# fegemo/palette-and-histo-gan

Measured on AMD Instinct MI355X. Metric: train images/sec (64x64x4 sprites), higher is better.
Workload: dtype bf16

## Files before the change

palette_and_histo_gan_amd/csrc/norm_act.hip:

```cpp
#include "p2p_common.hpp"
#include <stdlib.h>

#include <type_traits>

typedef __attribute__((__vector_size__(2 * sizeof(float)))) float f32x2;

__device__ __forceinline__ float act_apply(float y, int act, float alpha) {
    if (act == P2P_ACT_LEAKY) return y > 0.f ? y : alpha * y;
    if (act == P2P_ACT_RELU) return y > 0.f ? y : 0.f;
    return y;
}
__device__ __forceinline__ float act_slope(float a, int act, float alpha) {
    if (act == P2P_ACT_LEAKY) return a > 0.f ? 1.f : alpha;
    if (act == P2P_ACT_RELU) return a > 0.f ? 1.f : 0.f;
    return 1.f;
}

template <int VN> using mask_word = typename std::conditional<VN == 8, unsigned long long, unsigned>::type;
template <int VN>
__device__ __forceinline__ mask_word<VN> mask_vload(const unsigned char* m) { return *(const mask_word<VN>*)m; }
template <typename M>
__device__ __forceinline__ float mask_keep(M mk, int k) { return ((mk >> (8 * k)) & 0xff) ? 2.f : 0.f; }
template <int VN>
__device__ __forceinline__ void mask_vkeep(const unsigned char* m, float* keep) {
    const mask_word<VN> mk = mask_vload<VN>(m);
#pragma unroll
    for (int k = 0; k < VN; ++k) keep[k] = mask_keep(mk, k);
}

__device__ __forceinline__ float norm_xhat(float x, float mu, float rs) { return (x - mu) * rs; }

__device__ __forceinline__ float norm_affine(float x, float mu, float rs, float ga, float be) { return norm_xhat(x, mu, rs) * ga + be; }
__device__ __forceinline__ float drop_act(float y, bool drop, float keep, int act, float alpha) {
    if (drop) y *= keep;
    return act_apply(y, act, alpha);
}
__device__ __forceinline__ float fwd_elem(float x, float mu, float rs, float ga, float be, bool drop, float keep, int act, float alpha) {
    return drop_act(norm_affine(x, mu, rs, ga, be), drop, keep, act, alpha);
}

__device__ __forceinline__ float bwd_elem(bool norm, float xh, float ga, float be, float keep, float da, int act, float alpha) {
    float a = norm ? xh * ga + be : xh;
    a *= keep;
    return da * act_slope(a, act, alpha) * keep;
}
__device__ __forceinline__ float bwd_dx(float ga, float rs, float d, float m1, float xh, float m2) { return ga * rs * (d - m1 - xh * m2); }

template <typename T>
__device__ __forceinline__ float raw_load(const void* raw, int raw_kind, int nslabs, long long slab, long long e) {
    if (raw_kind == 1) return to_f32(((const T*)raw)[e]);
    float s = 0.f;
    const float* p = (const float*)raw + e;
    for (int k = 0; k < nslabs; ++k) s += p[(long long)k * slab];
    return to_f32(from_f32<T>(s));
}

template <typename T>
__global__ void norm_act_fwd_kernel(int H, int W, int C, int CB, const void* __restrict__ raw, int raw_kind,
// ... 151 lines not shown
#pragma unroll
        for (int u = 0; u < 4; ++u)
#pragma unroll
            for (int k = 0; k < VN; k += 4) r[u][k / 4] = *(const f32x4*)(p + (long long)(sIdx + u) * slab + k);
#pragma unroll
        for (int u = 0; u < 4; ++u)
#pragma unroll
            for (int k = 0; k < VN; k += 4) {
                v[k] += r[u][k / 4][0]; v[k + 1] += r[u][k / 4][1]; v[k + 2] += r[u][k / 4][2]; v[k + 3] += r[u][k / 4][3];
            }
    }
    return sIdx;
}

template <typename T, int SLABS = 1>
__device__ __forceinline__ void raw_vload(const void* raw, int raw_kind, int nslabs, long long slab, long long e, float* v) {
    constexpr int VN = VecOf<T>::N;
    if (SLABS == 0 || raw_kind == 1) { vload<T>((const T*)raw + e, v); return; }
#pragma unroll
    for (int k = 0; k < VN; ++k) v[k] = 0.f;
    const float* p = (const float*)raw + e;
    int sIdx = SLABS == 4 ? slabs4_add<VN>(p, slab, nslabs, v) : 0;
    for (; sIdx < nslabs; ++sIdx) {
#pragma unroll
        for (int k = 0; k < VN; k += 4) {
            f32x4 r = *(const f32x4*)(p + (long long)sIdx * slab + k);
            v[k] += r[0]; v[k + 1] += r[1]; v[k + 2] += r[2]; v[k + 3] += r[3];
        }
    }
#pragma unroll
    for (int k = 0; k < VN; ++k) v[k] = to_f32(from_f32<T>(v[k]));
}

template <typename T, int SLABS = 1>
__device__ __forceinline__ void gsrc_vload(const GSrc& g, long long pix, int c, float* v) {
    constexpr int VN = VecOf<T>::N;
    if (g.kind == 0) {
#pragma unroll
        for (int k = 0; k < VN; ++k) v[k] = 0.f;
        return;
    }
    long long e = pix * g.ld + g.coff + c;
    if (SLABS == 0 || g.kind == 1) { vload<T>((const T*)g.ptr + e, v); return; }
#pragma unroll
    for (int k = 0; k < VN; ++k) v[k] = 0.f;
    const float* p = (const float*)g.ptr + e;
    int sIdx = 0;
    if (SLABS == 4 && (g.slab & 3) == 0 && (e & 3) == 0 && ((uintptr_t)g.ptr & 15) == 0) sIdx = slabs4_add<VN>(p, g.slab, g.nslabs, v);
    for (; sIdx < g.nslabs; ++sIdx)
#pragma unroll
        for (int k = 0; k < VN; ++k) v[k] += p[(long long)sIdx * g.slab + k];
}

template <int VN> struct Coef { float mu[VN], rs[VN], ga[VN], be[VN]; };

template <int VN>
__device__ __forceinline__ void coef_load(const float* stats, const float* gamma, const float* beta, int n, int C, int c, Coef<VN>& co) {
#pragma unroll
    for (int k = 0; k < VN; ++k) {
        co.mu[k] = stats[((long long)n * C + c + k) * 2 + 0];
        co.rs[k] = stats[((long long)n * C + c + k) * 2 + 1];
        co.ga[k] = gamma[c + k];
        co.be[k] = beta[c + k];
    }
}

template <int VN>
__device__ __forceinline__ void coef_from_sums(const float* t1, const float* t2, const float* sh, int HW, float eps, const float* gamma,
                                               const float* beta, float* stats, bool write, int n, int C, int c, Coef<VN>& co) {
#pragma unroll
    for (int k = 0; k < VN; ++k) {
        const float m = t1[k] / (float)HW;
        const float var = fmaxf(t2[k] / (float)HW - m * m, 0.f);
        co.mu[k] = sh[k] + m;
        co.rs[k] = rsqrtf(var + eps);
        co.ga[k] = gamma[c + k];
        co.be[k] = beta[c + k];
        if (write) {
            stats[((long long)n * C + c + k) * 2 + 0] = co.mu[k];
            stats[((long long)n * C + c + k) * 2 + 1] = co.rs[k];
        }
    }
}

template <int VN> struct WgGeom {
    int VPP, PR, vid, pr, c;
    __device__ __forceinline__ WgGeom(int CG, int cg0)
        : VPP(CG / VN), PR(256 / VPP), vid(threadIdx.x % VPP), pr(threadIdx.x / VPP), c(cg0 + vid * VN) {}
};

template <int VN, bool TREE = false>
__device__ __forceinline__ void col_reduce2(float (*red)[2048], int CG, int PR, int vid, int pr, const float* s1,
                                            const float* s2, float* t1, float* t2) {
#pragma unroll
    for (int k = 0; k < VN; k += 4) {
        *(f32x4*)&red[0][pr * CG + vid * VN + k] = f32x4{s1[k], s1[k + 1], s1[k + 2], s1[k + 3]};
        *(f32x4*)&red[1][pr * CG + vid * VN + k] = f32x4{s2[k], s2[k + 1], s2[k + 2], s2[k + 3]};
    }
    __syncthreads();
    const int Q = 256 / CG;
    const int ch = threadIdx.x % CG, q = threadIdx.x / CG;
    float a = 0.f, b = 0.f;
    if (TREE) {
        float ra[VN], rb[VN];
#pragma unroll
        for (int j = 0; j < VN; ++j) { ra[j] = red[0][(q + j * Q) * CG + ch]; rb[j] = red[1][(q + j * Q) * CG + ch]; }
#pragma unroll
        for (int w = 1; w < VN; w *= 2)
#pragma unroll
            for (int j = 0; j < VN; j += 2 * w) { ra[j] += ra[j + w]; rb[j] += rb[j + w]; }
        a = ra[0]; b = rb[0];
    } else {
        for (int i = q; i < PR; i += Q) { a += red[0][i * CG + ch]; b += red[1][i * CG + ch]; }
    }
    __syncthreads();
    red[0][q * CG + ch] = a;
    red[1][q * CG + ch] = b;
    __syncthreads();
    if (threadIdx.x < CG) {
        float ta = 0.f, tb = 0.f;
        if (TREE) {
            float fa[8], fb[8];
#pragma unroll
            for (int g = 0; g < 8; ++g) {
                fa[g] = 0.f; fb[g] = 0.f;
                if (8 * g < Q) {
                    const float* pa = &red[0][8 * g * CG + threadIdx.x];
                    const float* pb = &red[1][8 * g * CG + threadIdx.x];
                    fa[g] = (pa[0] + pa[CG]) + (pa[2 * CG] + pa[3 * CG]);
                    fb[g] = (pb[0] + pb[CG]) + (pb[2 * CG] + pb[3 * CG]);
// ... 28 lines not shown
    }
}
template <int VN>
__device__ __forceinline__ void split_sum(const float* ws, float (*red)[2048], int n, int SP, int C, int cg0, int CG, int vid,
                                          float* t1, float* t2) {
    if (threadIdx.x < CG) {
        const int cc = cg0 + threadIdx.x;
        float a1 = 0.f, a2 = 0.f;
        for (int i = 0; i < SP; ++i) {
            const f32x2 v = *(const f32x2*)(ws + (((long long)n * SP + i) * C + cc) * 2);
            a1 += v[0]; a2 += v[1];
        }
        red[0][threadIdx.x] = a1;
        red[1][threadIdx.x] = a2;
    }
    __syncthreads();
#pragma unroll
    for (int k = 0; k < VN; ++k) { t1[k] = red[0][vid * VN + k]; t2[k] = red[1][vid * VN + k]; }
}

template <typename T>
__device__ __forceinline__ void tail_copy(T* dst, const T* src, int t0, int tail_vecs) {
    typedef typename VecOf<T>::type vec_t;
    for (int t = t0; t < tail_vecs; ++t) *(vec_t*)(dst + t * VecOf<T>::N) = *(const vec_t*)(src + t * VecOf<T>::N);
}

template <typename T, int MODE>
__global__ __launch_bounds__(256) void norm_act_fwd_vec(int H, int W, int C, int CG, const void* __restrict__ raw,
                                                        int raw_kind, int nslabs, long long slab,
                                                        const float* __restrict__ gamma, const float* __restrict__ beta,
                                                        float eps, int act, float alpha,
                                                        const unsigned char* __restrict__ mask, TView out,
                                                        T* __restrict__ raw_out, float* __restrict__ stats,
                                                        float* __restrict__ ws, int nslots, TView tail, int tail_vecs) {
    constexpr int VN = VecOf<T>::N;
    __shared__ __attribute__((aligned(16))) float red[2][2048];
    const int n = blockIdx.x;
    const int cg0 = blockIdx.y * CG;
    const int SP = gridDim.z, sp = blockIdx.z;
    const WgGeom<VN> wg(CG, cg0);
    const int PR = wg.PR, vid = wg.vid, pr = wg.pr, c = wg.c;
    const int HW = H * W;
    const int chunk = (HW + SP - 1) / SP;
    const int pb = sp * chunk, pe = min(HW, pb + chunk);
    const long long base = (long long)n * HW * C + c;
    Coef<VN> co;
    if (gamma) {
        float sh[VN], t1[VN], t2[VN];
        if (MODE != 3) raw_vload<T>(raw, raw_kind, nslabs, slab, base, sh);
        if (MODE < 2) {
            float s1[VN], s2[VN];
#pragma unroll
            for (int k = 0; k < VN; ++k) { s1[k] = 0.f; s2[k] = 0.f; }
            for (int p = pb + pr; p < pe; p += PR) {
                float x[VN];
                raw_vload<T>(raw, raw_kind, nslabs, slab, base + (long long)p * C, x);
#pragma unroll
                for (int k = 0; k < VN; ++k) { float d = x[k] - sh[k]; s1[k] += d; s2[k] += d * d; }
            }
            col_reduce2<VN>(red, CG, PR, vid, pr, s1, s2, t1, t2);
            if (MODE == 1) {
                if (pr == 0) split_store<VN>(ws, n, SP, sp, C, c, t1, t2);
                return;
            }
        } else if (MODE == 2) {
            split_sum<VN>(ws, red, n, SP, C, cg0, CG, vid, t1, t2);
        } else {
            if (threadIdx.x < CG) {
                const int cc = cg0 + threadIdx.x;
                float ms = 0.f;
                for (int i = 0; i < nslots; ++i) ms += ws[(((long long)n * nslots + i) * C + cc) * 2 + 0];
                const float mall = ms / (float)nslots;
                const float cnt = (float)HW / (float)nslots;
                float m2 = 0.f;
                for (int i = 0; i < nslots; ++i) {
                    float mi = ws[(((long long)n * nslots + i) * C + cc) * 2 + 0];
                    m2 += ws[(((long long)n * nslots + i) * C + cc) * 2 + 1] + cnt * (mi - mall) * (mi - mall);
                }
                red[0][threadIdx.x] = mall;
                red[1][threadIdx.x] = m2;
            }
            __syncthreads();
#pragma unroll
            for (int k = 0; k < VN; ++k) {
                sh[k] = red[0][vid * VN + k];
                t1[k] = 0.f;
                t2[k] = red[1][vid * VN + k];
            }
        }
        coef_from_sums<VN>(t1, t2, sh, HW, eps, gamma, beta, stats, pr == 0 && sp == 0, n, C, c, co);
    }
    if (raw_kind == 1 && !raw_out) {
        typedef typename VecOf<T>::type vec_t;
        constexpr int U = 4;
        const bool do_tail = tail_vecs && c + VN == C;
        for (int p0 = pb + pr; p0 < pe; p0 += PR * U) {
            vec_t xr[U], tr[U];
            unsigned long long mk[U];
#pragma unroll
            for (int u = 0; u < U; ++u) {
                const int p = p0 + u * PR;
                if (p < pe) {
                    const long long e = base + (long long)p * C;
                    xr[u] = *(const vec_t*)((const T*)raw + e);
                    if (mask) mk[u] = mask_vload<VN>(mask + e);
                    if (do_tail) {
                        const int yy = p / W, xx = p - yy * W;
                        tr[u] = *(const vec_t*)((const T*)tail.ptr + tail.off(n, yy, xx));
                    }
                }
            }
#pragma unroll
            for (int u = 0; u < U; ++u) {
                const int p = p0 + u * PR;
                if (p >= pe) continue;
                vec_t o;
#pragma unroll
                for (int k = 0; k < VN; ++k)
                {
                    const float xv = to_f32((T)xr[u][k]);
                    const float y = gamma ? norm_affine(xv, co.mu[k], co.rs[k], co.ga[k], co.be[k]) : xv;
                    o[k] = from_f32<T>(drop_act(y, mask, mask ? mask_keep(mk[u], k) : 1.f, act, alpha));
                }
                const int yy = p / W, xx = p - yy * W;
                T* op = (T*)out.ptr + out.off(n, yy, xx);
                *(vec_t*)(op + c) = o;
                if (do_tail) {
                    *(vec_t*)(op + C) = tr[u];
                    tail_copy<T>(op + C, (const T*)tail.ptr + tail.off(n, yy, xx), 1, tail_vecs);
                }
            }
        }
        return;
    }
    for (int p = pb + pr; p < pe; p += PR) {
        long long e = base + (long long)p * C;
        float x[VN], keep[VN];
        raw_vload<T>(raw, raw_kind, nslabs, slab, e, x);
        if (raw_out) vstore<T>(raw_out + e, x);
        if (mask) mask_vkeep<VN>(mask + e, keep);
#pragma unroll
        for (int k = 0; k < VN; ++k) {
            const float y = gamma ? norm_affine(x[k], co.mu[k], co.rs[k], co.ga[k], co.be[k]) : x[k];
            x[k] = drop_act(y, mask, mask ? keep[k] : 1.f, act, alpha);
        }
        int yy = p / W, xx = p - yy * W;
        T* op = (T*)out.ptr + out.off(n, yy, xx);
        vstore<T>(op + c, x);
        if (tail_vecs && c + VN == C) tail_copy<T>(op + C, (const T*)tail.ptr + tail.off(n, yy, xx), 0, tail_vecs);
    }
}

template <typename T, int MODE>
__global__ __launch_bounds__(256) void norm_act_bwd_vec(int H, int W, int C, int CG, const T* __restrict__ raw,
                                                        const float* __restrict__ stats, const float* __restrict__ gamma,
                                                        const float* __restrict__ beta, int act, float alpha,
                                                        const unsigned char* __restrict__ mask, GSrc g1, GSrc g2,
                                                        TView draw, float* __restrict__ dgamma_part,
                                                        float* __restrict__ dbeta_part, float* __restrict__ ws) {
    constexpr int VN = VecOf<T>::N;
    __shared__ __attribute__((aligned(16))) float red[2][2048];
    const int n = blockIdx.x;
    const int cg0 = blockIdx.y * CG;
    const int SP = gridDim.z, sp = blockIdx.z;
    const WgGeom<VN> wg(CG, cg0);
    const int PR = wg.PR, vid = wg.vid, pr = wg.pr, c = wg.c;
    const int HW = H * W;
    const int chunk = (HW + SP - 1) / SP;
    const int pb = sp * chunk, pe = min(HW, pb + chunk);
    const long long pix0 = (long long)n * HW;
    const long long base = pix0 * C + c;
    Coef<VN> co;
    coef_load<VN>(stats, gamma, beta, n, C, c, co);
    auto dyhat = [&](int p, float* d, float* xh) {
        long long e = base + (long long)p * C;
        float x[VN], a1[VN], a2[VN], keep[VN];
        vload<T>(raw + e, x);
        gsrc_vload<T>(g1, pix0 + p, c, a1);
        gsrc_vload<T>(g2, pix0 + p, c, a2);
        if (mask) mask_vkeep<VN>(mask + e, keep);
#pragma unroll
        for (int k = 0; k < VN; ++k) {
            xh[k] = norm_xhat(x[k], co.mu[k], co.rs[k]);
            d[k] = bwd_elem(true, xh[k], co.ga[k], co.be[k], mask ? keep[k] : 1.f, a1[k] + a2[k], act, alpha);
        }
    };
    float t1[VN], t2[VN];
    if (MODE != 2) {
        float s1[VN], s2[VN];
#pragma unroll
        for (int k = 0; k < VN; ++k) { s1[k] = 0.f; s2[k] = 0.f; }
        for (int p = pb + pr; p < pe; p += PR) {
            float d[VN], xh[VN];
            dyhat(p, d, xh);
#pragma unroll
            for (int k = 0; k < VN; ++k) { s1[k] += d[k]; s2[k] += d[k] * xh[k]; }
        }
        col_reduce2<VN>(red, CG, PR, vid, pr, s1, s2, t1, t2);
        if (MODE == 1) {
            if (pr == 0) split_store<VN>(ws, n, SP, sp, C, c, t1, t2);
            return;
        }
    } else {
        split_sum<VN>(ws, red, n, SP, C, cg0, CG, vid, t1, t2);
    }
    float m1[VN], m2[VN];
#pragma unroll
    for (int k = 0; k < VN; ++k) {
        if (pr == 0 && sp == 0) {
            dbeta_part[(long long)n * C + c + k] = t1[k];
            dgamma_part[(long long)n * C + c + k] = t2[k];
        }
        m1[k] = t1[k] / (float)HW;
        m2[k] = t2[k] / (float)HW;
    }
    for (int p = pb + pr; p < pe; p += PR) {
        float d[VN], xh[VN];
        dyhat(p, d, xh);
#pragma unroll
        for (int k = 0; k < VN; ++k) d[k] = bwd_dx(co.ga[k], co.rs[k], d[k], m1[k], xh[k], m2[k]);
        int yy = p / W, xx = p - yy * W;
        vstore<T>((T*)draw.ptr + draw.off(n, yy, xx) + c, d);
    }
}

__device__ __forceinline__ void reg_block(int C, int CG, int& n, int& cg0) {
    const int ncg = C / CG;
    const int lin = blockIdx.x;
    n = ((lin >> 3) / ncg) * 8 + (lin & 7);
    cg0 = ((lin >> 3) % ncg) * CG;
}
static inline unsigned reg_grid(int N, int C, int CG) { return (unsigned)(((N + 7) / 8) * 8 * (C / CG)); }

template <typename T, int PPL, int SLABS>
__global__ __launch_bounds__(256) void norm_act_bwd_reg(int N, int HW, int W, int C, int CG, const T* __restrict__ raw,
                                                        const float* __restrict__ stats, const float* __restrict__ gamma,
                                                        const float* __restrict__ beta, int act, float alpha,
                                                        const unsigned char* __restrict__ mask, GSrc g1, GSrc g2, TView draw,
                                                        float* __restrict__ dgamma_part, float* __restrict__ dbeta_part) {
    constexpr int VN = VecOf<T>::N;
    typedef typename VecOf<T>::type vec_t;
    __shared__ __attribute__((aligned(16))) float red[2][2048];
    int n, cg0;
    reg_block(C, CG, n, cg0);
    if (n >= N) return;
    const WgGeom<VN> wg(CG, cg0);
    const int PR = wg.PR, vid = wg.vid, pr = wg.pr, c = wg.c;
    const long long pix0 = (long long)n * HW;
    const long long base = pix0 * C + c;
    Coef<VN> co;
    coef_load<VN>(stats, gamma, beta, n, C, c, co);
    vec_t xr[PPL];
    float d[PPL][VN];
    float s1[VN], s2[VN];
#pragma unroll
    for (int k = 0; k < VN; ++k) { s1[k] = 0.f; s2[k] = 0.f; }
#pragma unroll
    for (int i = 0; i < PPL; ++i) {
        const int p = pr + i * PR;
        if (p < HW) {
            const long long e = base + (long long)p * C;
            float a1[VN], a2[VN], keep[VN];
            xr[i] = *(const vec_t*)(raw + e);
            gsrc_vload<T, SLABS>(g1, pix0 + p, c, a1);
            gsrc_vload<T, SLABS>(g2, pix0 + p, c, a2);
            if (mask) mask_vkeep<VN>(mask + e, keep);
#pragma unroll
            for (int k = 0; k < VN; ++k) {
                const float xh = norm_xhat(to_f32((T)xr[i][k]), co.mu[k], co.rs[k]);
                d[i][k] = bwd_elem(true, xh, co.ga[k], co.be[k], mask ? keep[k] : 1.f, a1[k] + a2[k], act, alpha);
                s1[k] += d[i][k];
                s2[k] += d[i][k] * xh;
            }
        } else {
#pragma unroll
            for (int k = 0; k < VN; ++k) d[i][k] = 0.f;
        }
    }
    float t1[VN], t2[VN];
    col_reduce2<VN>(red, CG, PR, vid, pr, s1, s2, t1, t2);
    float m1[VN], m2[VN];
#pragma unroll
    for (int k = 0; k < VN; ++k) {
        if (pr == 0) {
            dbeta_part[(long long)n * C + c + k] = t1[k];
            dgamma_part[(long long)n * C + c + k] = t2[k];
        }
        m1[k] = t1[k] / (float)HW;
        m2[k] = t2[k] / (float)HW;
    }
#pragma unroll
    for (int i = 0; i < PPL; ++i) {
        const int p = pr + i * PR;
        if (p >= HW) continue;
        float r[VN];
#pragma unroll
        for (int k = 0; k < VN; ++k) {
            const float xh = norm_xhat(to_f32((T)xr[i][k]), co.mu[k], co.rs[k]);
            r[k] = bwd_dx(co.ga[k], co.rs[k], d[i][k], m1[k], xh, m2[k]);
        }
        const int yy = p / W, xx = p - yy * W;
        vstore<T>((T*)draw.ptr + draw.off(n, yy, xx) + c, r);
    }
}

static inline int norm_bwd_reg_geom(int Neff, int HW, int C, int vn, int& ppl_out, bool fwd = false) {
    static int max_hw[2] = {-1, -1};
    if (max_hw[fwd] < 0) { const char* e = getenv(fwd ? "P2P_NORM_FWD_REG" : "P2P_NORM_BWD_REG"); max_hw[fwd] = e ? atoi(e) : 4096; }
    static int min_wgs = -1;
    if (min_wgs < 0) { const char* e = getenv("P2P_NORM_REG_WGS"); min_wgs = e ? atoi(e) : 512; }
    ppl_out = 0;
    if (HW > max_hw[fwd]) return 0;
    int pick = 0, pick_ppl = 0;
    for (int CG = 64; CG >= vn; CG >>= 1) {
        if (CG > C || C % CG) continue;
        const int pr = 256 / (CG / vn);
        int ppl = (HW + pr - 1) / pr;
        ppl = ppl <= 1 ? 1 : (ppl <= 2 ? 2 : (ppl <= 4 ? 4 : 8));
        if ((long long)ppl * pr < HW) continue;
        pick = CG; pick_ppl = ppl;
        if ((long long)Neff * (C / CG) >= min_wgs) break;
    }
    ppl_out = pick_ppl;
    return pick;
}

template <typename T, int PPL, int SLABS>
__global__ __launch_bounds__(256) void norm_act_fwd_reg(int N, int HW, int W, int C, int CG, const void* __restrict__ raw,
                                                        int raw_kind, int nslabs, long long slab,
                                                        const float* __restrict__ gamma, const float* __restrict__ beta,
                                                        float eps, int act, float alpha,
                                                        const unsigned char* __restrict__ mask, TView out,
                                                        T* __restrict__ raw_out, float* __restrict__ stats) {
    constexpr int VN = VecOf<T>::N;
    __shared__ __attribute__((aligned(16))) float red[2][2048];
    int n, cg0;
    reg_block(C, CG, n, cg0);
    if (n >= N) return;
    const WgGeom<VN> wg(CG, cg0);
    const int PR = wg.PR, vid = wg.vid, pr = wg.pr, c = wg.c;
    const long long base = (long long)n * HW * C + c;
    float x[PPL][VN], sh[VN], s1[VN], s2[VN];
    unsigned long long mk[PPL];
    raw_vload<T, SLABS>(raw, raw_kind, nslabs, slab, base, sh);
#pragma unroll
    for (int i = 0; i < PPL; ++i) {
        const int p = pr + i * PR;
        mk[i] = 0;
        if (p < HW) {
            const long long e = base + (long long)p * C;
            raw_vload<T, SLABS>(raw, raw_kind, nslabs, slab, e, x[i]);
            if (mask) mk[i] = mask_vload<VN>(mask + e);
        } else {
#pragma unroll
            for (int k = 0; k < VN; ++k) x[i][k] = 0.f;
        }
    }
#pragma unroll
    for (int k = 0; k < VN; ++k) { s1[k] = 0.f; s2[k] = 0.f; }
#pragma unroll
    for (int i = 0; i < PPL; ++i)
        if (pr + i * PR < HW)
#pragma unroll
            for (int k = 0; k < VN; ++k) { const float d = x[i][k] - sh[k]; s1[k] += d; s2[k] += d * d; }
    float t1[VN], t2[VN];
    Coef<VN> co;
    col_reduce2<VN, VN == 4>(red, CG, PR, vid, pr, s1, s2, t1, t2);
    coef_from_sums<VN>(t1, t2, sh, HW, eps, gamma, beta, stats, pr == 0, n, C, c, co);
#pragma unroll
    for (int i = 0; i < PPL; ++i) {
        const int p = pr + i * PR;
        if (p >= HW) continue;
        if (raw_out) vstore<T>(raw_out + base + (long long)p * C, x[i]);
        float y[VN];
#pragma unroll
        for (int k = 0; k < VN; ++k) y[k] = fwd_elem(x[i][k], co.mu[k], co.rs[k], co.ga[k], co.be[k], mask, mask_keep(mk[i], k), act, alpha);
        const int yy = p / W, xx = p - yy * W;
        vstore<T>((T*)out.ptr + out.off(n, yy, xx) + c, y);
    }
}

template <typename T, int PPL, int SLABS>
__global__ __launch_bounds__(256) void norm_act_fwd_small(int HW, int W, int C, int lgG, long long items, const void* __restrict__ raw,
                                                          int raw_kind, int nslabs, long long slab, const float* __restrict__ gamma,
                                                          const float* __restrict__ beta, float eps, int act, float alpha,
                                                          const unsigned char* __restrict__ mask, TView out,
                                                          T* __restrict__ raw_out, float* __restrict__ stats) {
    constexpr int VN = VecOf<T>::N;
    const int G = 1 << lgG;
    const long long gid = (long long)blockIdx.x * 256 + threadIdx.x;
    const long long item = gid >> lgG;
    const int g = (int)(gid & (G - 1));
    if (item >= items) return;
    const int cvn = C / VN;
    const int n = (int)(item / cvn), c = (int)(item - (long long)n * cvn) * VN;
    const long long base = (long long)n * HW * C + c;
    float x[PPL][VN];
#pragma unroll
    for (int i = 0; i < PPL; ++i) {
        const int p = g + i * G;
        if (p < HW) raw_vload<T, SLABS>(raw, raw_kind, nslabs, slab, base + (long long)p * C, x[i]);
        else {
#pragma unroll
            for (int k = 0; k < VN; ++k) x[i][k] = 0.f;
        }
    }
    float mu[VN], rs[VN];
    if (gamma) {
#pragma unroll
        for (int k = 0; k < VN; ++k) {
            float s = 0.f;
#pragma unroll
            for (int i = 0; i < PPL; ++i) s += x[i][k];
            for (int o = G >> 1; o > 0; o >>= 1) s += __shfl_xor(s, o, 64);
            mu[k] = s / (float)HW;
            float q = 0.f;
#pragma unroll
            for (int i = 0; i < PPL; ++i) {
                const float d = (g + i * G < HW) ? x[i][k] - mu[k] : 0.f;
                q += d * d;
            }
            for (int o = G >> 1; o > 0; o >>= 1) q += __shfl_xor(q, o, 64);
            rs[k] = rsqrtf(q / (float)HW + eps);
            if (g == 0) {
                stats[((long long)n * C + c + k) * 2 + 0] = mu[k];
                stats[((long long)n * C + c + k) * 2 + 1] = rs[k];
            }
        }
    }
#pragma unroll
    for (int i = 0; i < PPL; ++i) {
        const int p = g + i * G;
        if (p >= HW) continue;
        const long long e = base + (long long)p * C;
        float keep[VN], y[VN];
        if (raw_out) vstore<T>(raw_out + e, x[i]);
        if (mask) mask_vkeep<VN>(mask + e, keep);
#pragma unroll
        for (int k = 0; k < VN; ++k) {
            const float v = gamma ? norm_affine(x[i][k], mu[k], rs[k], gamma[c + k], beta[c + k]) : x[i][k];
            y[k] = drop_act(v, mask, mask ? keep[k] : 1.f, act, alpha);
        }
        const int yy = p / W, xx = p - yy * W;
        vstore<T>((T*)out.ptr + out.off(n, yy, xx) + c, y);
    }
}

template <typename T, int PPL, int SLABS>
__global__ __launch_bounds__(256) void norm_act_bwd_small(int HW, int W, int C, int lgG, long long items, const T* __restrict__ raw,
                                                          const float* __restrict__ stats, const float* __restrict__ gamma,
                                                          const float* __restrict__ beta, int act, float alpha,
                                                          const unsigned char* __restrict__ mask, GSrc g1, GSrc g2, TView draw,
                                                          float* __restrict__ dgamma_part, float* __restrict__ dbeta_part) {
    constexpr int VN = VecOf<T>::N;
    const int G = 1 << lgG;
    const long long gid = (long long)blockIdx.x * 256 + threadIdx.x;
    const long long item = gid >> lgG;
    const int g = (int)(gid & (G - 1));
    if (item >= items) return;
    const int cvn = C / VN;
    const int n = (int)(item / cvn), c = (int)(item - (long long)n * cvn) * VN;
    const long long pix0 = (long long)n * HW, base = pix0 * C + c;
    Coef<VN> co;
    coef_load<VN>(stats, gamma, beta, n, C, c, co);
    float d[PPL][VN], xh[PPL][VN];
#pragma unroll
    for (int i = 0; i < PPL; ++i) {
        const int p = g + i * G;
        if (p < HW) {
            const long long e = base + (long long)p * C;
            float x[VN], a1[VN], a2[VN], keep[VN];
            vload<T>(raw + e, x);
            gsrc_vload<T, SLABS>(g1, pix0 + p, c, a1);
            gsrc_vload<T, SLABS>(g2, pix0 + p, c, a2);
            if (mask) mask_vkeep<VN>(mask + e, keep);
#pragma unroll
            for (int k = 0; k < VN; ++k) {
                xh[i][k] = norm_xhat(x[k], co.mu[k], co.rs[k]);
                d[i][k] = bwd_elem(true, xh[i][k], co.ga[k], co.be[k], mask ? keep[k] : 1.f, a1[k] + a2[k], act, alpha);
            }
        } else {
#pragma unroll
            for (int k = 0; k < VN; ++k) { d[i][k] = 0.f; xh[i][k] = 0.f; }
        }
    }
    float m1[VN], m2[VN];
#pragma unroll
    for (int k = 0; k < VN; ++k) {
        float t1 = 0.f, t2 = 0.f;
#pragma unroll
        for (int i = 0; i < PPL; ++i) { t1 += d[i][k]; t2 += d[i][k] * xh[i][k]; }
        for (int o = G >> 1; o > 0; o >>= 1) { t1 += __shfl_xor(t1, o, 64); t2 += __shfl_xor(t2, o, 64); }
        if (g == 0) {
            dbeta_part[(long long)n * C + c + k] = t1;
            dgamma_part[(long long)n * C + c + k] = t2;
        }
        m1[k] = t1 / (float)HW;
        m2[k] = t2 / (float)HW;
    }
#pragma unroll
    for (int i = 0; i < PPL; ++i) {
        const int p = g + i * G;
        if (p >= HW) continue;
        float r[VN];
#pragma unroll
        for (int k = 0; k < VN; ++k) r[k] = bwd_dx(co.ga[k], co.rs[k], d[i][k], m1[k], xh[i][k], m2[k]);
        const int yy = p / W, xx = p - yy * W;
        vstore<T>((T*)draw.ptr + draw.off(n, yy, xx) + c, r);
    }
}

static inline void small_geom(int HW, int& lgG, int& ppl) {
    lgG = 0;
    while ((1 << lgG) < HW && lgG < 4) ++lgG;
    const int G = 1 << lgG;
    const int need = (HW + G - 1) / G;
    ppl = need <= 1 ? 1 : (need <= 2 ? 2 : 4);
}

__global__ __launch_bounds__(256) void colsum_batched_kernel(const float* __restrict__ part, const int* __restrict__ table,
                                                             float* __restrict__ out) {
    __shared__ f32x4 red[16][16];
    const int* t = table + 4 * blockIdx.y;
    const int poff = t[0], rows = t[1], cols = t[2], ooff = t[3];
    const int cq = threadIdx.x & 15, rg = threadIdx.x >> 4;
    const int c = blockIdx.x * 64 + cq * 4;
    if (blockIdx.x * 64 >= cols) return;
    f32x4 s = {0.f, 0.f, 0.f, 0.f};
    if (c < cols) {
        const float* p = part + (long long)poff + c;
        if ((cols & 3) == 0 && (poff & 3) == 0) {
#pragma unroll 4
            for (int r = rg; r < rows; r += 16) s += *(const f32x4*)(p + (long long)r * cols);
        } else {
            for (int r = rg; r < rows; r += 16)
                for (int k = 0; k < 4; ++k)
                    if (c + k < cols) s[k] += p[(long long)r * cols + k];
        }
    }
    red[rg][cq] = s;
    __syncthreads();
    if (rg == 0 && c < cols) {
        f32x4 tsum = red[0][cq];
#pragma unroll
// ... 66 lines not shown
            return p2p_check_launch("p2p_act_bwd");
        }
    }
    long long total = (long long)N * H * W * C;
    long long blocks = (total + 255) / 256;
    if (blocks > 4096) blocks = 4096;
    P2P_DISPATCH_DTYPE(dtype, (act_bwd_kernel<T><<<dim3((unsigned)blocks), 256, 0, (hipStream_t)stream>>>(
                                  N, H, W, C, make_view(act_out), make_gsrc(g1), make_gsrc(g2), alpha, make_view(draw))));
    return p2p_check_launch("p2p_act_bwd");
}

__global__ void colsum_kernel(const float* __restrict__ part, int rows, int cols, float scale, float* __restrict__ out) {
    int c = blockIdx.x * blockDim.x + threadIdx.x;
    if (c >= cols) return;
    float s = 0.f;
    for (int r = 0; r < rows; ++r) s += part[(long long)r * cols + c];
    out[c] = s * scale;
}

static inline int pick_cb(int C) { return C >= 64 ? 64 : (C >= 32 ? 32 : (C >= 16 ? 16 : (C >= 8 ? 8 : (C >= 4 ? 4 : (C >= 2 ? 2 : 1))))); }

struct NormRoute { int form, ppl, cg, lgG, sp, slabs; };

static int norm_route_code(const NormRoute& r) {
    int lg = 0;
    while ((1 << lg) < r.cg) ++lg;
    return P2P_NORM_ROUTE(r.form, r.ppl, r.slabs, lg);
}

struct NSplit {
    int sp;
    bool two_pass;
    bool geom256;
    int nslots;
};
static NSplit nsplit_decode(int nsplit) {
    NSplit s = {1, false, false, 0};
    if (nsplit > 0) {
        s.sp = (nsplit & 0xff) < 1 ? 1 : (nsplit & 0xff);
        s.two_pass = (nsplit & 0x100) != 0;
        s.geom256 = (nsplit & 0x200) != 0;
    } else if (nsplit < 0) {
        s.nslots = -nsplit;
    }
    return s;
}

static int vec_cg(int C, int vn) {
    int CG = C > 64 ? 64 : C;
    while (C % CG) CG -= vn;
    return 256 % (CG / vn) == 0 ? CG : 0;
}

template <int V> using ic = std::integral_constant<int, V>;
template <typename F>
static void dispatch_slabs(bool slabs, F&& f) {
    if (slabs) f(ic<4>{}); else f(ic<0>{});
}
template <int MAXPPL, typename F>
static void dispatch_ppl_slabs(int ppl, bool slabs, F&& f) {
    dispatch_slabs(slabs, [&](auto S) {
        if (ppl == 1) f(ic<1>{}, S);
        else if (ppl == 2) f(ic<2>{}, S);
        else if (MAXPPL == 4 || ppl == 4) f(ic<4>{}, S);
        else if constexpr (MAXPPL == 8) f(ic<8>{}, S);
    });
}
template <typename K, typename... A>
static void launch256(bool last, K kernel, dim3 grid, hipStream_t st, A... args) {
    if (last) P2P_LAUNCH_LAST(kernel, grid, dim3(256), 0, st, args...);
    else hipLaunchKernelGGL(kernel, grid, dim3(256), 0, st, args...);
}

static NormRoute norm_fwd_route(int N, int HW, int C, int vn, bool vec, bool has_gamma, bool has_tail, int raw_kind, const NSplit& ns,
                                bool has_ws, long long ws_bytes) {
    NormRoute r = {P2P_NORM_FORM_SCALAR, 0, 0, 0, 1, 0};
    if (vec && HW <= 16) {
        r.form = P2P_NORM_FORM_SMALL;
        r.slabs = raw_kind == 2;
        small_geom(HW, r.lgG, r.ppl);
        return r;
    }
    if (vec && has_gamma && !has_tail && !ns.nslots && !ns.two_pass) {
        int ppl = 0;
        const int rcg = norm_bwd_reg_geom(ns.geom256 ? 256 : N, HW, C, vn, ppl, true);
        if (rcg) {
            r.form = P2P_NORM_FORM_REG; r.cg = rcg; r.ppl = ppl; r.slabs = raw_kind == 2;
            return r;
        }
    }
    const int CG = vec ? vec_cg(C, vn) : 0;
    if (CG) {
        const int prr = 256 / (CG / vn);
        int sp = ns.sp;
        while (sp > 1 && (HW + sp - 1) / sp < prr) sp >>= 1;
        r.cg = CG;
        if (ns.nslots && has_gamma && has_ws) { r.form = P2P_NORM_FORM_VEC3; return r; }
        if (!has_ws || (long long)N * sp * C * 2 * 4 > ws_bytes) sp = has_gamma ? 1 : sp;
        r.sp = sp;
        r.form = (sp == 1 || !has_gamma) ? P2P_NORM_FORM_VEC0 : P2P_NORM_FORM_VEC12;
    }
    return r;
}

static int norm_act_fwd_impl(int dtype, int N, int H, int W, int C, const void* raw, int raw_kind, int nslabs,
                             long long slab_stride, const float* gamma, const float* beta, float eps, int act,
                             float alpha, const unsigned char* mask, const p2p_tensor* out, void* raw_out,
// ... 280 lines not shown
```

Before: 132,500.

## Batch pixel loads in norm/act kernels to raise memory-level parallelism

```diff
diff --git a/palette_and_histo_gan_amd/csrc/norm_act.hip b/palette_and_histo_gan_amd/csrc/norm_act.hip
--- a/palette_and_histo_gan_amd/csrc/norm_act.hip
+++ b/palette_and_histo_gan_amd/csrc/norm_act.hip
@@ -4,6 +4,7 @@
 #include <type_traits>
 
 typedef __attribute__((__vector_size__(2 * sizeof(float)))) float f32x2;
+template <int V> using ic = std::integral_constant<int, V>;
 
 __device__ __forceinline__ float act_apply(float y, int act, float alpha) {
     if (act == P2P_ACT_LEAKY) return y > 0.f ? y : alpha * y;
@@ -261,6 +262,184 @@
         for (int k = 0; k < VN; ++k) v[k] += p[(long long)sIdx * g.slab + k];
 }
 
+template <typename T, int NP>
+__device__ __forceinline__ void vload_n(const T* p, const long long* e, const bool* live, long long e0, typename VecOf<T>::type* r) {
+#pragma unroll
+    for (int j = 0; j < NP; ++j) r[j] = *(const typename VecOf<T>::type*)(p + (live[j] ? e[j] : e0));
+}
+template <typename T>
+__device__ __forceinline__ void vunpack(const typename VecOf<T>::type& r, float* v) {
+#pragma unroll
+    for (int k = 0; k < VecOf<T>::N; ++k) v[k] = to_f32((T)r[k]);
+}
+template <int VN, int NP>
+__device__ __forceinline__ void mask_vload_n(const unsigned char* mask, const long long* e, const bool* live, long long e0, mask_word<VN>* mk) {
+#pragma unroll
+    for (int j = 0; j < NP; ++j) mk[j] = 0;
+    if (mask) {
+#pragma unroll
+        for (int j = 0; j < NP; ++j) mk[j] = mask_vload<VN>(mask + (live[j] ? e[j] : e0));
+    }
+}
+
+__device__ __forceinline__ void loads_landed() {
+    asm volatile("" ::: "memory");
+    __builtin_amdgcn_s_waitcnt(0x0f70);
+}
+
+template <int VN, int J, int S, bool AL>
+__device__ __forceinline__ void slabs_trip(const float* p, long long slab, int s0, int nslabs, const long long* e, float (*v)[VN]) {
+    float r[S][J][VN];
+#pragma unroll
+    for (int u = 0; u < S; ++u) {
+        const float* q = p + (long long)(u == 0 ? s0 : min(s0 + u, nslabs - 1)) * slab;
+#pragma unroll
+        for (int j = 0; j < J; ++j) {
+            if (AL) {
+#pragma unroll
+                for (int k = 0; k < VN; k += 4) {
+                    const f32x4 t = *(const f32x4*)(q + e[j] + k);
+                    r[u][j][k] = t[0]; r[u][j][k + 1] = t[1]; r[u][j][k + 2] = t[2]; r[u][j][k + 3] = t[3];
+                }
+            } else {
+#pragma unroll
+                for (int k = 0; k < VN; ++k) r[u][j][k] = q[e[j] + k];
+            }
+        }
+    }
+#pragma unroll
+    for (int u = 0; u < S; ++u) {
+        const bool there = u == 0 || s0 + u < nslabs;
+#pragma unroll
+        for (int j = 0; j < J; ++j)
+#pragma unroll
+            for (int k = 0; k < VN; ++k) v[j][k] += there ? r[u][j][k] : 0.f;
+    }
+}
+template <int VN, int NP, int INFLIGHT, bool AL>
+__device__ __forceinline__ void slabs_add_n(const float* p, long long slab, int nslabs, const long long* e, const bool* live, long long e0,
+                                            float (*v)[VN]) {
+    constexpr int J = NP * VN <= INFLIGHT ? NP : INFLIGHT / VN;
+    constexpr int S = INFLIGHT / (J * VN) > 8 ? 8 : INFLIGHT / (J * VN);
+    static_assert(J >= 1 && S >= 1, "slabs_add_n: INFLIGHT holds at least one pixel");
+    long long ec[J];
+#pragma unroll
+    for (int j = 0; j < J; ++j) {
+        ec[j] = live[j] ? e[j] : e0;
+#pragma unroll
+        for (int k = 0; k < VN; ++k) v[j][k] = 0.f;
+    }
+    for (int s0 = 0; s0 < nslabs; s0 += S) slabs_trip<VN, J, S, AL>(p, slab, s0, nslabs, ec, v);
+#pragma unroll
+    for (int j = 0; j < J; ++j)
+#pragma unroll
+        for (int k = 0; k < VN; ++k) v[j][k] = live[j] ? v[j][k] : 0.f;
+    if constexpr (J < NP) slabs_add_n<VN, NP - J, INFLIGHT, AL>(p, slab, nslabs, e + J, live + J, e0, v + J);
+}
+
+template <typename T, int NP, int SLABS, int INFLIGHT = (NP * VecOf<T>::N >= 32 ? 32 : 64)>
+__device__ __forceinline__ void raw_vload_n(const void* raw, int raw_kind, int nslabs, long long slab, const long long* e, const bool* live,
+                                            long long e0, float (*x)[VecOf<T>::N]) {
+    constexpr int VN = VecOf<T>::N;
+    const bool dense = SLABS == 0 || raw_kind == 1;
+    typename VecOf<T>::type r[NP];
+    if (dense) vload_n<T, NP>((const T*)raw, e, live, e0, r);
+    else slabs_add_n<VN, NP, INFLIGHT, true>((const float*)raw, slab, nslabs, e, live, e0, x);
+    loads_landed();
+#pragma unroll
+    for (int j = 0; j < NP; ++j)
+        if (live[j]) {
+            if (dense) {
+                vunpack<T>(r[j], x[j]);
+            } else {
+#pragma unroll
+                for (int k = 0; k < VN; ++k) x[j][k] = to_f32(from_f32<T>(x[j][k]));
+            }
+        }
+}
+
+template <typename T, int NP, int SLABS, int INFLIGHT = (NP * VecOf<T>::N >= 32 ? 32 : 64)>
+struct BwdPixels {
+    static constexpr int VN = VecOf<T>::N;
+    typedef typename VecOf<T>::type vec_t;
+    vec_t x[NP];
+    mask_word<VN> mk[NP];
+    vec_t gr[2][NP];
+    float gs[2][SLABS ? NP : 1][VN];
+
+    __device__ __forceinline__ void load_dense(int w, const GSrc& g, const long long* pix, const bool* live, long long pix0, int c) {
+        if (g.kind == 1 || (SLABS == 0 && g.kind)) {
+            long long e[NP];
+#pragma unroll
+            for (int j = 0; j < NP; ++j) e[j] = pix[j] * g.ld + g.coff + c;
+            vload_n<T, NP>((const T*)g.ptr, e, live, pix0 * g.ld + g.coff + c, gr[w]);
+        } else {
+#pragma unroll
+            for (int j = 0; j < NP; ++j) gr[w][j] = vec_t{};
+        }
+    }
+    __device__ __forceinline__ void load(const T* raw, const unsigned char* mask, const GSrc& g1, const GSrc& g2, int C, int c,
+                                         const long long* pix, const bool* live, long long pix0) {
+        long long e[NP];
+#pragma unroll
+        for (int j = 0; j < NP; ++j) e[j] = pix[j] * C + c;
+        vload_n<T, NP>(raw, e, live, pix0 * C + c, x);
+        mask_vload_n<VN, NP>(mask, e, live, pix0 * C + c, mk);
+        load_dense(0, g1, pix, live, pix0, c);
+        load_dense(1, g2, pix, live, pix0, c);
+        if constexpr (SLABS != 0) {
+#pragma nounroll
+            for (int w = 0; w < 2; ++w) {
+                const GSrc& g = w ? g2 : g1;
+                if (g.kind != 2) continue;
+                float acc[NP][VN];
+#pragma unroll
+                for (int j = 0; j < NP; ++j) e[j] = pix[j] * g.ld + g.coff + c;
+                const long long e0 = pix0 * g.ld + g.coff + c;
+                if ((g.slab & 3) == 0 && (g.ld & 3) == 0 && (g.coff & 3) == 0 && ((uintptr_t)g.ptr & 15) == 0)
+                    slabs_add_n<VN, NP, INFLIGHT, true>((const float*)g.ptr, g.slab, g.nslabs, e, live, e0, acc);
+                else
+                    slabs_add_n<VN, NP, INFLIGHT, false>((const float*)g.ptr, g.slab, g.nslabs, e, live, e0, acc);
+#pragma unroll
+                for (int j = 0; j < NP; ++j)
+#pragma unroll
+                    for (int k = 0; k < VN; ++k) {
+                        if (w == 0) gs[0][j][k] = acc[j][k];
+                        else gs[1][j][k] = acc[j][k];
+                    }
+            }
+        }
+        loads_landed();
+        if constexpr (SLABS != 0) {
+            if (g1.kind != 2) {
+#pragma unroll
+                for (int j = 0; j < NP; ++j) vunpack<T>(gr[0][j], gs[0][j]);
+            }
+            if (g2.kind != 2) {
+#pragma unroll
+                for (int j = 0; j < NP; ++j) vunpack<T>(gr[1][j], gs[1][j]);
+            }
+#pragma unroll
+            for (int j = 0; j < NP; ++j)
+#pragma unroll
+                for (int k = 0; k < VN; ++k) gs[0][j][k] = gs[0][j][k] + gs[1][j][k];
+        }
+    }
+    __device__ __forceinline__ void grad(int i, float* da) const {
+        if constexpr (SLABS == 0) {
+            float a1[VN], a2[VN];
+            vunpack<T>(gr[0][i], a1);
+            vunpack<T>(gr[1][i], a2);
+#pragma unroll
+            for (int k = 0; k < VN; ++k) da[k] = a1[k] + a2[k];
+        } else {
+#pragma unroll
+            for (int k = 0; k < VN; ++k) da[k] = gs[0][i][k];
+        }
+    }
+    __device__ __forceinline__ float keep(bool has_mask, int i, int k) const { return has_mask ? mask_keep(mk[i], k) : 1.f; }
+};
+
 template <int VN> struct Coef { float mu[VN], rs[VN], ga[VN], be[VN]; };
 
 template <int VN>
@@ -275,16 +454,16 @@
 }
 
 template <int VN>
-__device__ __forceinline__ void coef_from_sums(const float* t1, const float* t2, const float* sh, int HW, float eps, const float* gamma,
-                                               const float* beta, float* stats, bool write, int n, int C, int c, Coef<VN>& co) {
+__device__ __forceinline__ void coef_from_sums(const float* t1, const float* t2, const float* sh, int HW, float eps, const float* ga,
+                                               const float* be, float* stats, bool write, int n, int C, int c, Coef<VN>& co) {
 #pragma unroll
     for (int k = 0; k < VN; ++k) {
         const float m = t1[k] / (float)HW;
         const float var = fmaxf(t2[k] / (float)HW - m * m, 0.f);
         co.mu[k] = sh[k] + m;
         co.rs[k] = rsqrtf(var + eps);
-        co.ga[k] = gamma[c + k];
-        co.be[k] = beta[c + k];
+        co.ga[k] = ga[k];
+        co.be[k] = be[k];
         if (write) {
             stats[((long long)n * C + c + k) * 2 + 0] = co.mu[k];
             stats[((long long)n * C + c + k) * 2 + 1] = co.rs[k];
@@ -419,12 +598,27 @@
             float s1[VN], s2[VN];
 #pragma unroll
             for (int k = 0; k < VN; ++k) { s1[k] = 0.f; s2[k] = 0.f; }
-            for (int p = pb + pr; p < pe; p += PR) {
-                float x[VN];
-                raw_vload<T>(raw, raw_kind, nslabs, slab, base + (long long)p * C, x);
-#pragma unroll
-                for (int k = 0; k < VN; ++k) { float d = x[k] - sh[k]; s1[k] += d; s2[k] += d * d; }
-            }
+            auto trip = [&](auto S, auto UU, int p0) {
+                constexpr int U = decltype(UU)::value;
+                float x[U][VN];
+                long long e[U];
+                bool live[U];
+#pragma unroll
+                for (int u = 0; u < U; ++u) { e[u] = base + (long long)(p0 + u * PR) * C; live[u] = true; }
+                raw_vload_n<T, U, decltype(S)::value, 32>(raw, raw_kind, nslabs, slab, e, live, base, x);
+#pragma unroll
+                for (int u = 0; u < U; ++u)
+#pragma unroll
+                    for (int k = 0; k < VN; ++k) { float d = x[u][k] - sh[k]; s1[k] += d; s2[k] = fmaf(d, d, s2[k]); }
+            };
+            auto trips = [&](auto S, auto UU) {
+                constexpr int U = decltype(UU)::value;
+                int p0 = pb + pr;
+                for (; p0 + (U - 1) * PR < pe; p0 += PR * U) trip(S, UU, p0);
+                for (; p0 < pe; p0 += PR) trip(S, ic<1>{}, p0);
+            };
+            if (raw_kind == 1) trips(ic<0>{}, ic<4>{});
+            else trips(ic<1>{}, ic<2>{});
             col_reduce2<VN>(red, CG, PR, vid, pr, s1, s2, t1, t2);
             if (MODE == 1) {
                 if (pr == 0) split_store<VN>(ws, n, SP, sp, C, c, t1, t2);
@@ -455,7 +649,10 @@
                 t2[k] = red[1][vid * VN + k];
             }
         }
-        coef_from_sums<VN>(t1, t2, sh, HW, eps, gamma, beta, stats, pr == 0 && sp == 0, n, C, c, co);
+        float ga[VN], be[VN];
+#pragma unroll
+        for (int k = 0; k < VN; ++k) { ga[k] = gamma[c + k]; be[k] = beta[c + k]; }
+        coef_from_sums<VN>(t1, t2, sh, HW, eps, ga, be, stats, pr == 0 && sp == 0, n, C, c, co);
     }
     if (raw_kind == 1 && !raw_out) {
         typedef typename VecOf<T>::type vec_t;
@@ -500,22 +697,39 @@
         }
         return;
     }
-    for (int p = pb + pr; p < pe; p += PR) {
-        long long e = base + (long long)p * C;
-        float x[VN], keep[VN];
-        raw_vload<T>(raw, raw_kind, nslabs, slab, e, x);
-        if (raw_out) vstore<T>(raw_out + e, x);
-        if (mask) mask_vkeep<VN>(mask + e, keep);
-#pragma unroll
-        for (int k = 0; k < VN; ++k) {
-            const float y = gamma ? norm_affine(x[k], co.mu[k], co.rs[k], co.ga[k], co.be[k]) : x[k];
-            x[k] = drop_act(y, mask, mask ? keep[k] : 1.f, act, alpha);
-        }
-        int yy = p / W, xx = p - yy * W;
-        T* op = (T*)out.ptr + out.off(n, yy, xx);
-        vstore<T>(op + c, x);
-        if (tail_vecs && c + VN == C) tail_copy<T>(op + C, (const T*)tail.ptr + tail.off(n, yy, xx), 0, tail_vecs);
-    }
+    auto trip = [&](auto S, auto UU, int p0) {
+        constexpr int U = decltype(UU)::value;
+        float x[U][VN];
+        long long e[U];
+        bool live[U];
+        mask_word<VN> mk[U];
+#pragma unroll
+        for (int u = 0; u < U; ++u) { e[u] = base + (long long)(p0 + u * PR) * C; live[u] = true; }
+        mask_vload_n<VN, U>(mask, e, live, base, mk);
+        raw_vload_n<T, U, decltype(S)::value, 32>(raw, raw_kind, nslabs, slab, e, live, base, x);
+#pragma unroll
+        for (int u = 0; u < U; ++u) {
+            const int p = p0 + u * PR;
+            if (raw_out) vstore<T>(raw_out + e[u], x[u]);
+#pragma unroll
+            for (int k = 0; k < VN; ++k) {
+                const float y = gamma ? norm_affine(x[u][k], co.mu[k], co.rs[k], co.ga[k], co.be[k]) : x[u][k];
+                x[u][k] = drop_act(y, mask, mask ? mask_keep(mk[u], k) : 1.f, act, alpha);
+            }
+            int yy = p / W, xx = p - yy * W;
+            T* op = (T*)out.ptr + out.off(n, yy, xx);
+            vstore<T>(op + c, x[u]);
+            if (tail_vecs && c + VN == C) tail_copy<T>(op + C, (const T*)tail.ptr + tail.off(n, yy, xx), 0, tail_vecs);
+        }
+    };
+    auto trips = [&](auto S, auto UU) {
+        constexpr int U = decltype(UU)::value;
+        int p0 = pb + pr;
+        for (; p0 + (U - 1) * PR < pe; p0 += PR * U) trip(S, UU, p0);
+        for (; p0 < pe; p0 += PR) trip(S, ic<1>{}, p0);
+    };
+    if (raw_kind == 1) trips(ic<0>{}, ic<4>{});
+    else trips(ic<1>{}, ic<2>{});
 }
 
 template <typename T, int MODE>
@@ -536,11 +750,38 @@
     const int chunk = (HW + SP - 1) / SP;
     const int pb = sp * chunk, pe = min(HW, pb + chunk);
     const long long pix0 = (long long)n * HW;
-    const long long base = pix0 * C + c;
     Coef<VN> co;
     coef_load<VN>(stats, gamma, beta, n, C, c, co);
+    const bool has_mask = mask != nullptr;
+    auto trip = [&](auto S, auto UU, int p0, auto&& use) {
+        constexpr int U = decltype(UU)::value;
+        BwdPixels<T, U, decltype(S)::value, 32> px;
+        long long pix[U];
+        bool live[U];
+#pragma unroll
+        for (int u = 0; u < U; ++u) { pix[u] = pix0 + p0 + u * PR; live[u] = true; }
+        px.load(raw, mask, g1, g2, C, c, pix, live, pix0);
+#pragma unroll
+        for (int u = 0; u < U; ++u) {
+            float x[VN], da[VN], d[VN], xh[VN];
+            vunpack<T>(px.x[u], x);
+            px.grad(u, da);
+#pragma unroll
+            for (int k = 0; k < VN; ++k) {
+                xh[k] = norm_xhat(x[k], co.mu[k], co.rs[k]);
+                d[k] = bwd_elem(true, xh[k], co.ga[k], co.be[k], px.keep(has_mask, u, k), da[k], act, alpha);
+            }
+            use(p0 + u * PR, d, xh);
+        }
+    };
+    auto trips = [&](auto S, auto UU, auto&& use) {
+        constexpr int U = decltype(UU)::value;
+        int p0 = pb + pr;
+        for (; p0 + (U - 1) * PR < pe; p0 += PR * U) trip(S, UU, p0, use);
+        for (; p0 < pe; p0 += PR) trip(S, ic<1>{}, p0, use);
+    };
     auto dyhat = [&](int p, float* d, float* xh) {
-        long long e = base + (long long)p * C;
+        long long e = pix0 * C + c + (long long)p * C;
         float x[VN], a1[VN], a2[VN], keep[VN];
         vload<T>(raw + e, x);
         gsrc_vload<T>(g1, pix0 + p, c, a1);
@@ -552,17 +793,31 @@
             d[k] = bwd_elem(true, xh[k], co.ga[k], co.be[k], mask ? keep[k] : 1.f, a1[k] + a2[k], act, alpha);
         }
     };
+    auto pixels = [&](auto&& use) {
+        if constexpr (VN == 4) {
+            for (int p = pb + pr; p < pe; p += PR) {
+                float d[VN], xh[VN];
+                dyhat(p, d, xh);
+                use(p, d, xh);
+            }
+        } else {
+            if (g1.kind == 2 || g2.kind == 2) trips(ic<1>{}, ic<1>{}, use);
+            else trips(ic<0>{}, ic<2>{}, use);
+        }
+    };
     float t1[VN], t2[VN];
     if (MODE != 2) {
         float s1[VN], s2[VN];
 #pragma unroll
         for (int k = 0; k < VN; ++k) { s1[k] = 0.f; s2[k] = 0.f; }
-        for (int p = pb + pr; p < pe; p += PR) {
-            float d[VN], xh[VN];
-            dyhat(p, d, xh);
-#pragma unroll
-            for (int k = 0; k < VN; ++k) { s1[k] += d[k]; s2[k] += d[k] * xh[k]; }
-        }
+        pixels([&](int, const float* d, const float* xh) {
+#pragma unroll
+            for (int k = 0; k < VN; ++k) {
+                s1[k] += d[k];
+                if (VN == 4) s2[k] += d[k] * xh[k];
+                else s2[k] = fmaf(d[k], xh[k], s2[k]);
+            }
+        });
         col_reduce2<VN>(red, CG, PR, vid, pr, s1, s2, t1, t2);
         if (MODE == 1) {
             if (pr == 0) split_store<VN>(ws, n, SP, sp, C, c, t1, t2);
@@ -581,14 +836,13 @@
         m1[k] = t1[k] / (float)HW;
         m2[k] = t2[k] / (float)HW;
     }
-    for (int p = pb + pr; p < pe; p += PR) {
-        float d[VN], xh[VN];
-        dyhat(p, d, xh);
-#pragma unroll
-        for (int k = 0; k < VN; ++k) d[k] = bwd_dx(co.ga[k], co.rs[k], d[k], m1[k], xh[k], m2[k]);
+    pixels([&](int p, const float* d, const float* xh) {
+        float r[VN];
+#pragma unroll
+        for (int k = 0; k < VN; ++k) r[k] = bwd_dx(co.ga[k], co.rs[k], d[k], m1[k], xh[k], m2[k]);
         int yy = p / W, xx = p - yy * W;
-        vstore<T>((T*)draw.ptr + draw.off(n, yy, xx) + c, d);
-    }
+        vstore<T>((T*)draw.ptr + draw.off(n, yy, xx) + c, r);
+    });
 }
 
 __device__ __forceinline__ void reg_block(int C, int CG, int& n, int& cg0) {
@@ -614,30 +868,31 @@
     const WgGeom<VN> wg(CG, cg0);
     const int PR = wg.PR, vid = wg.vid, pr = wg.pr, c = wg.c;
     const long long pix0 = (long long)n * HW;
-    const long long base = pix0 * C + c;
     Coef<VN> co;
     coef_load<VN>(stats, gamma, beta, n, C, c, co);
-    vec_t xr[PPL];
+    BwdPixels<T, PPL, SLABS> px;
+    long long pix[PPL];
+    bool live[PPL];
+#pragma unroll
+    for (int i = 0; i < PPL; ++i) { pix[i] = pix0 + pr + i * PR; live[i] = pr + i * PR < HW; }
+    px.load(raw, mask, g1, g2, C, c, pix, live, pix0);
+    const vec_t (&xr)[PPL] = px.x;
+    const bool has_mask = mask != nullptr;
     float d[PPL][VN];
     float s1[VN], s2[VN];
 #pragma unroll
     for (int k = 0; k < VN; ++k) { s1[k] = 0.f; s2[k] = 0.f; }
 #pragma unroll
     for (int i = 0; i < PPL; ++i) {
-        const int p = pr + i * PR;
-        if (p < HW) {
-            const long long e = base + (long long)p * C;
-            float a1[VN], a2[VN], keep[VN];
-            xr[i] = *(const vec_t*)(raw + e);
-            gsrc_vload<T, SLABS>(g1, pix0 + p, c, a1);
-            gsrc_vload<T, SLABS>(g2, pix0 + p, c, a2);
-            if (mask) mask_vkeep<VN>(mask + e, keep);
+        if (live[i]) {
+            float da[VN];
+            px.grad(i, da);
 #pragma unroll
             for (int k = 0; k < VN; ++k) {
                 const float xh = norm_xhat(to_f32((T)xr[i][k]), co.mu[k], co.rs[k]);
-                d[i][k] = bwd_elem(true, xh, co.ga[k], co.be[k], mask ? keep[k] : 1.f, a1[k] + a2[k], act, alpha);
+                d[i][k] = bwd_elem(true, xh, co.ga[k], co.be[k], px.keep(has_mask, i, k), da[k], act, alpha);
                 s1[k] += d[i][k];
-                s2[k] += d[i][k] * xh;
+                s2[k] = fmaf(d[i][k], xh, s2[k]);
             }
         } else {
 #pragma unroll
@@ -707,33 +962,35 @@
     const WgGeom<VN> wg(CG, cg0);
     const int PR = wg.PR, vid = wg.vid, pr = wg.pr, c = wg.c;
     const long long base = (long long)n * HW * C + c;
-    float x[PPL][VN], sh[VN], s1[VN], s2[VN];
-    unsigned long long mk[PPL];
-    raw_vload<T, SLABS>(raw, raw_kind, nslabs, slab, base, sh);
+    float x[PPL + 1][VN], s1[VN], s2[VN], ga[VN], be[VN];
+    long long e[PPL + 1];
+    bool live[PPL + 1];
+    mask_word<VN> mk[PPL];
 #pragma unroll
     for (int i = 0; i < PPL; ++i) {
-        const int p = pr + i * PR;
-        mk[i] = 0;
-        if (p < HW) {
-            const long long e = base + (long long)p * C;
-            raw_vload<T, SLABS>(raw, raw_kind, nslabs, slab, e, x[i]);
-            if (mask) mk[i] = mask_vload<VN>(mask + e);
-        } else {
-#pragma unroll
-            for (int k = 0; k < VN; ++k) x[i][k] = 0.f;
-        }
-    }
+        e[i] = base + (long long)(pr + i * PR) * C;
+        live[i] = pr + i * PR < HW;
+#pragma unroll
+        for (int k = 0; k < VN; ++k) x[i][k] = 0.f;
+    }
+    e[PPL] = base;
+    live[PPL] = true;
+    mask_vload_n<VN, PPL>(mask, e, live, base, mk);
+#pragma unroll
+    for (int k = 0; k < VN; ++k) { ga[k] = gamma[c + k]; be[k] = beta[c + k]; }
+    raw_vload_n<T, PPL + 1, SLABS, ((PPL + 1) * VN > 64 ? (PPL + 1) * VN : 64)>(raw, raw_kind, nslabs, slab, e, live, base, x);
+    const float (&sh)[VN] = x[PPL];
 #pragma unroll
     for (int k = 0; k < VN; ++k) { s1[k] = 0.f; s2[k] = 0.f; }
 #pragma unroll
     for (int i = 0; i < PPL; ++i)
-        if (pr + i * PR < HW)
-#pragma unroll
-            for (int k = 0; k < VN; ++k) { const float d = x[i][k] - sh[k]; s1[k] += d; s2[k] += d * d; }
+        if (live[i])
+#pragma unroll
+            for (int k = 0; k < VN; ++k) { const float d = x[i][k] - sh[k]; s1[k] += d; s2[k] = fmaf(d, d, s2[k]); }
     float t1[VN], t2[VN];
     Coef<VN> co;
     col_reduce2<VN, VN == 4>(red, CG, PR, vid, pr, s1, s2, t1, t2);
-    coef_from_sums<VN>(t1, t2, sh, HW, eps, gamma, beta, stats, pr == 0, n, C, c, co);
+    coef_from_sums<VN>(t1, t2, sh, HW, eps, ga, be, stats, pr == 0, n, C, c, co);
 #pragma unroll
     for (int i = 0; i < PPL; ++i) {
         const int p = pr + i * PR;
@@ -763,15 +1020,18 @@
     const int n = (int)(item / cvn), c = (int)(item - (long long)n * cvn) * VN;
     const long long base = (long long)n * HW * C + c;
     float x[PPL][VN];
+    long long e[PPL];
+    bool live[PPL];
+    mask_word<VN> mk[PPL];
 #pragma unroll
     for (int i = 0; i < PPL; ++i) {
-        const int p = g + i * G;
-        if (p < HW) raw_vload<T, SLABS>(raw, raw_kind, nslabs, slab, base + (long long)p * C, x[i]);
-        else {
-#pragma unroll
-            for (int k = 0; k < VN; ++k) x[i][k] = 0.f;
-        }
-    }
+        e[i] = base + (long long)(g + i * G) * C;
+        live[i] = g + i * G < HW;
+#pragma unroll
+        for (int k = 0; k < VN; ++k) x[i][k] = 0.f;
+    }
+    mask_vload_n<VN, PPL>(mask, e, live, base, mk);
+    raw_vload_n<T, PPL, SLABS>(raw, raw_kind, nslabs, slab, e, live, base, x);
     float mu[VN], rs[VN];
     if (gamma) {
 #pragma unroll
@@ -799,14 +1059,12 @@
     for (int i = 0; i < PPL; ++i) {
         const int p = g + i * G;
         if (p >= HW) continue;
-        const long long e = base + (long long)p * C;
-        float keep[VN], y[VN];
-        if (raw_out) vstore<T>(raw_out + e, x[i]);
-        if (mask) mask_vkeep<VN>(mask + e, keep);
+        float y[VN];
+        if (raw_out) vstore<T>(raw_out + e[i], x[i]);
 #pragma unroll
         for (int k = 0; k < VN; ++k) {
             const float v = gamma ? norm_affine(x[i][k], mu[k], rs[k], gamma[c + k], beta[c + k]) : x[i][k];
-            y[k] = drop_act(v, mask, mask ? keep[k] : 1.f, act, alpha);
+            y[k] = drop_act(v, mask, mask ? mask_keep(mk[i], k) : 1.f, act, alpha);
         }
         const int yy = p / W, xx = p - yy * W;
         vstore<T>((T*)out.ptr + out.off(n, yy, xx) + c, y);
@@ -827,24 +1085,27 @@
     if (item >= items) return;
     const int cvn = C / VN;
     const int n = (int)(item / cvn), c = (int)(item - (long long)n * cvn) * VN;
-    const long long pix0 = (long long)n * HW, base = pix0 * C + c;
+    const long long pix0 = (long long)n * HW;
     Coef<VN> co;
     coef_load<VN>(stats, gamma, beta, n, C, c, co);
+    BwdPixels<T, PPL, SLABS> px;
+    long long pix[PPL];
+    bool live[PPL];
+#pragma unroll
+    for (int i = 0; i < PPL; ++i) { pix[i] = pix0 + g + i * G; live[i] = g + i * G < HW; }
+    px.load(raw, mask, g1, g2, C, c, pix, live, pix0);
+    const bool has_mask = mask != nullptr;
     float d[PPL][VN], xh[PPL][VN];
 #pragma unroll
     for (int i = 0; i < PPL; ++i) {
-        const int p = g + i * G;
-        if (p < HW) {
-            const long long e = base + (long long)p * C;
-            float x[VN], a1[VN], a2[VN], keep[VN];
-            vload<T>(raw + e, x);
-            gsrc_vload<T, SLABS>(g1, pix0 + p, c, a1);
-            gsrc_vload<T, SLABS>(g2, pix0 + p, c, a2);
-            if (mask) mask_vkeep<VN>(mask + e, keep);
+        if (live[i]) {
+            float x[VN], da[VN];
+            vunpack<T>(px.x[i], x);
+            px.grad(i, da);
 #pragma unroll
             for (int k = 0; k < VN; ++k) {
                 xh[i][k] = norm_xhat(x[k], co.mu[k], co.rs[k]);
-                d[i][k] = bwd_elem(true, xh[i][k], co.ga[k], co.be[k], mask ? keep[k] : 1.f, a1[k] + a2[k], act, alpha);
+                d[i][k] = bwd_elem(true, xh[i][k], co.ga[k], co.be[k], px.keep(has_mask, i, k), da[k], act, alpha);
             }
         } else {
 #pragma unroll
@@ -856,7 +1117,7 @@
     for (int k = 0; k < VN; ++k) {
         float t1 = 0.f, t2 = 0.f;
 #pragma unroll
-        for (int i = 0; i < PPL; ++i) { t1 += d[i][k]; t2 += d[i][k] * xh[i][k]; }
+        for (int i = 0; i < PPL; ++i) { t1 += d[i][k]; t2 = fmaf(d[i][k], xh[i][k], t2); }
         for (int o = G >> 1; o > 0; o >>= 1) { t1 += __shfl_xor(t1, o, 64); t2 += __shfl_xor(t2, o, 64); }
         if (g == 0) {
             dbeta_part[(long long)n * C + c + k] = t1;
@@ -1029,7 +1290,6 @@
     return 256 % (CG / vn) == 0 ? CG : 0;
 }
 
-template <int V> using ic = std::integral_constant<int, V>;
 template <typename F>
 static void dispatch_slabs(bool slabs, F&& f) {
     if (slabs) f(ic<4>{}); else f(ic<0>{});
```

Result: no change. 131,800 (-0.5%).
